# qope/SIPP

Hardware: AMD Instinct MI355X
Metric: SIPP proof-gen wall-clock + pairings-aggregated/sec, n=128 (the 3 STARK sub-proofs, hardened G1/G2 AIRs; outer plonky2 proof not included) (higher is better)
Workload: dtype u64; 1 GPU; n=128 SIPP instance per GPU: G1ExpStark 127 IO (N=2^16, W+P+Q=1176), G2ExpStark 127 IO (N=2^16, 2314), Fq12ExpStark 14 IO (N=2^13, 7970); IO records on host -> 3 flat proofs on host, the 3 sub-proofs on 3 concurrent HIP streams; parallelism=1 independent SIPP instance(s), one per GPU, no collective

## Files before the change

### sipp_amd/csrc/trace.hip

```cpp
#include <algorithm>

#include "air_prog.hpp"
#include "air_tables.h"
#include "ctx.hpp"
#include "fq.hpp"

namespace {

using fq::Fq;
using fq::Fq2;

template <int EXT>
struct Fld;
template <>
struct Fld<1> {
    using T = Fq;
    static __device__ __forceinline__ T add(const T& a, const T& b) { return fq::add(a, b); }
    static __device__ __forceinline__ T sub(const T& a, const T& b) { return fq::sub(a, b); }
    static __device__ __forceinline__ T mul(const T& a, const T& b) { return fq::mul(a, b); }
    static __device__ __forceinline__ T sqr(const T& a) { return fq::sqr(a); }
    static __device__ __forceinline__ T inv(const T& a) { return fq::inv(a); }
    static __device__ __forceinline__ bool is_zero(const T& a) { return fq::is_zero(a); }
    static __device__ __forceinline__ T load(const uint32_t* w) {
        Fq r;
#pragma unroll
        for (int i = 0; i < 8; i++) r.l[i] = w[i];
        return fq::to_mont(r);
    }
};
template <>
struct Fld<2> {
    using T = Fq2;
    static __device__ __forceinline__ T add(const T& a, const T& b) { return fq::add(a, b); }
    static __device__ __forceinline__ T sub(const T& a, const T& b) { return fq::sub(a, b); }
    static __device__ __forceinline__ T mul(const T& a, const T& b) { return fq::mul(a, b); }
    static __device__ __forceinline__ T sqr(const T& a) { return fq::sqr(a); }
    static __device__ __forceinline__ T inv(const T& a) { return fq::inv(a); }
    static __device__ __forceinline__ bool is_zero(const T& a) { return fq::is_zero(a); }
    static __device__ __forceinline__ T load(const uint32_t* w) {
        return Fq2{Fld<1>::load(w), Fld<1>::load(w + 8)};
    }
};

__device__ __forceinline__ Fq one_of(Fq*) { return fq::one_m(); }
__device__ __forceinline__ Fq2 one_of(Fq2*) { return Fq2{fq::one_m(), fq::zero()}; }

template <int EXT>
__device__ __forceinline__ bool point_on_curve(const uint32_t* w) {
    using F = Fld<EXT>;
    const auto x = F::load(w), y = F::load(w + 8 * EXT);
    const auto d = F::sub(F::sqr(y), F::mul(F::sqr(x), x));
    const Fq three = fq::small_m(3);
    if constexpr (EXT == 1) {
        return fq::is_zero(fq::sub(d, three));
    } else {
        const Fq nine = fq::small_m(9);
        const Fq re = fq::sub(fq::mul(nine, d.c0), d.c1), im = fq::add(d.c0, fq::mul(nine, d.c1));
        return fq::is_zero(fq::sub(re, three)) && fq::is_zero(im);
    }
}


template <int EXT>
struct Jac {
    typename Fld<EXT>::T x, y, z;
};

template <int EXT>
__device__ __forceinline__ Jac<EXT> jac_dbl(const Jac<EXT>& p) {
    using F = Fld<EXT>;
    auto A = F::sqr(p.x), B = F::sqr(p.y), C = F::sqr(B);
    auto t = F::add(p.x, B);
    auto D = F::sub(F::sub(F::sqr(t), A), C);
    D = F::add(D, D);
    auto E = F::add(F::add(A, A), A);
    auto Fv = F::sqr(E);
    Jac<EXT> r;
    r.x = F::sub(Fv, F::add(D, D));
    auto C8 = F::add(C, C);
    C8 = F::add(C8, C8);
    C8 = F::add(C8, C8);
    r.y = F::sub(F::mul(E, F::sub(D, r.x)), C8);
    auto yz = F::mul(p.y, p.z);
    r.z = F::add(yz, yz);
    return r;
}

template <int EXT>
__device__ __forceinline__ Jac<EXT> jac_add(const Jac<EXT>& p, const Jac<EXT>& q) {
    using F = Fld<EXT>;
    auto z1z1 = F::sqr(p.z), z2z2 = F::sqr(q.z);
    auto u1 = F::mul(p.x, z2z2), u2 = F::mul(q.x, z1z1);
    auto s1 = F::mul(F::mul(p.y, q.z), z2z2), s2 = F::mul(F::mul(q.y, p.z), z1z1);
    auto h = F::sub(u2, u1);
    auto rr = F::sub(s2, s1);
    if (F::is_zero(h)) {
        if (F::is_zero(rr)) return jac_dbl<EXT>(p);
        Jac<EXT> inf;
        inf.x = one_of((typename F::T*)nullptr);
        inf.y = inf.x;
        inf.z = F::sub(inf.x, inf.x);
        return inf;
    }
    auto i = F::add(h, h);
    i = F::sqr(i);
    auto j = F::mul(h, i);
    rr = F::add(rr, rr);
    auto v = F::mul(u1, i);
    Jac<EXT> r;
    r.x = F::sub(F::sub(F::sqr(rr), j), F::add(v, v));
    auto s1j = F::mul(s1, j);
    r.y = F::sub(F::mul(rr, F::sub(v, r.x)), F::add(s1j, s1j));
    auto zz = F::add(p.z, q.z);
    r.z = F::mul(F::sub(F::sub(F::sqr(zz), z1z1), z2z2), h);
    return r;
}


template <int EXT>
struct RowPts {
    Jac<EXT> R, P;
};

template <int EXT>
__device__ __forceinline__ bool jac_is_inf(const Jac<EXT>& p) { return Fld<EXT>::is_zero(p.z); }

template <int EXT>
__device__ __forceinline__ Jac<EXT> jac_add_id(const Jac<EXT>& p, const Jac<EXT>& q) {
    if (jac_is_inf<EXT>(p)) return q;
    if (jac_is_inf<EXT>(q)) return p;
    return jac_add<EXT>(p, q);
}

__device__ __forceinline__ void lds_put(Fq* dst, const Fq& v) {
    uint4* d = reinterpret_cast<uint4*>(dst);
    d[0] = make_uint4(v.l[0], v.l[1], v.l[2], v.l[3]);
    d[1] = make_uint4(v.l[4], v.l[5], v.l[6], v.l[7]);
}
__device__ __forceinline__ Fq lds_get(const Fq* src) {
    const uint4* d = reinterpret_cast<const uint4*>(src);
    const uint4 a = d[0], b = d[1];
    Fq v;
    v.l[0] = a.x; v.l[1] = a.y; v.l[2] = a.z; v.l[3] = a.w;
    v.l[4] = b.x; v.l[5] = b.y; v.l[6] = b.z; v.l[7] = b.w;
    return v;
}

template <int NT>
__device__ __forceinline__ void par_level(Fq* s_op, Fq* s_pr, int sub, const Fq (&a)[NT], const Fq (&b)[NT], Fq (&p)[NT]) {
#pragma unroll
    for (int t = 0; t < NT; t++) {
        lds_put(s_op + 2 * t, a[t]);
        lds_put(s_op + 2 * t + 1, b[t]);
    }
    __syncthreads();
    const int task = sub < NT ? sub : NT - 1;
    const Fq x = lds_get(s_op + 2 * task), y = lds_get(s_op + 2 * task + 1);
    lds_put(s_pr + sub, fq::mul(x, y));
    __syncthreads();
#pragma unroll
    for (int t = 0; t < NT; t++) p[t] = lds_get(s_pr + t);
}

__device__ __forceinline__ Jac<1> jac_dbl_par(const Jac<1>& P, Fq* s_op, Fq* s_pr, int sub) {
    Fq p1[3], p2[3], p3[1];
    {
        const Fq a[3] = {P.x, P.y, P.y}, b[3] = {P.x, P.y, P.z};
        par_level<3>(s_op, s_pr, sub, a, b, p1);
    }
    const Fq A = p1[0], B = p1[1];
    const Fq U = fq::add(P.x, B), E = fq::add(fq::add(A, A), A);
    {
        const Fq a[3] = {B, U, E};
        par_level<3>(s_op, s_pr, sub, a, a, p2);
    }
    const Fq C = p2[0];
    Fq D = fq::sub(fq::sub(p2[1], A), C);
    D = fq::add(D, D);
    Jac<1> r;
    r.x = fq::sub(p2[2], fq::add(D, D));
    {
        const Fq a[1] = {E}, b[1] = {fq::sub(D, r.x)};
        par_level<1>(s_op, s_pr, sub, a, b, p3);
    }
    Fq C8 = fq::add(C, C);
    C8 = fq::add(C8, C8);
    C8 = fq::add(C8, C8);
    r.y = fq::sub(p3[0], C8);
    r.z = fq::add(p1[2], p1[2]);
    return r;
}

__device__ __forceinline__ Jac<2> jac_dbl_par(const Jac<2>& P, Fq* s_op, Fq* s_pr, int sub) {
    Fq p1[7], p2[6], p3[3];
    {
        const Fq a[7] = {fq::add(P.x.c0, P.x.c1), P.x.c0, fq::add(P.y.c0, P.y.c1), P.y.c0, P.y.c0, P.y.c1,
                         fq::add(P.y.c0, P.y.c1)};
        const Fq b[7] = {fq::sub(P.x.c0, P.x.c1), P.x.c1, fq::sub(P.y.c0, P.y.c1), P.y.c1, P.z.c0, P.z.c1,
                         fq::add(P.z.c0, P.z.c1)};
        par_level<7>(s_op, s_pr, sub, a, b, p1);
    }
    const Fq2 A{p1[0], fq::add(p1[1], p1[1])}, B{p1[2], fq::add(p1[3], p1[3])};
    const Fq2 YZ{fq::sub(p1[4], p1[5]), fq::sub(fq::sub(p1[6], p1[4]), p1[5])};
    const Fq2 U = fq::add(P.x, B), E = fq::add(fq::add(A, A), A);
    {
        const Fq a[6] = {fq::add(B.c0, B.c1), B.c0, fq::add(U.c0, U.c1), U.c0, fq::add(E.c0, E.c1), E.c0};
        const Fq b[6] = {fq::sub(B.c0, B.c1), B.c1, fq::sub(U.c0, U.c1), U.c1, fq::sub(E.c0, E.c1), E.c1};
        par_level<6>(s_op, s_pr, sub, a, b, p2);
    }
    const Fq2 C{p2[0], fq::add(p2[1], p2[1])}, S{p2[2], fq::add(p2[3], p2[3])}, Fv{p2[4], fq::add(p2[5], p2[5])};
    Fq2 D = fq::sub(fq::sub(S, A), C);
    D = fq::add(D, D);
    Jac<2> r;
    r.x = fq::sub(Fv, fq::add(D, D));
    const Fq2 Wd = fq::sub(D, r.x);
    {
        const Fq a[3] = {E.c0, E.c1, fq::add(E.c0, E.c1)}, b[3] = {Wd.c0, Wd.c1, fq::add(Wd.c0, Wd.c1)};
        par_level<3>(s_op, s_pr, sub, a, b, p3);
    }
    const Fq2 EW{fq::sub(p3[0], p3[1]), fq::sub(fq::sub(p3[2], p3[0]), p3[1])};
    Fq2 C8 = fq::add(C, C);
    C8 = fq::add(C8, C8);
    C8 = fq::add(C8, C8);
    r.y = fq::sub(EW, C8);
    r.z = fq::add(YZ, YZ);
    return r;
}

template <int EXT, int G>
__global__ void __launch_bounds__(64) curve_dbl_par_kernel(const uint32_t* __restrict__ ios, uint32_t num_io, uint32_t ppi,
                                                          RowPts<EXT>* __restrict__ rows) {
    using F = Fld<EXT>;
    using T = typename F::T;
    constexpr int GPB = 64 / G;
    __shared__ Fq s_op[GPB][14], s_pr[GPB][G];
    const int grp = threadIdx.x / G, sub = threadIdx.x % G;
    uint32_t io = blockIdx.x * GPB + grp;
    const bool live = io < num_io && sub == 0;
    if (io >= num_io) io = num_io - 1;
    const uint32_t* rec = ios + (size_t)io * ppi;
    const int w = 8 * EXT;
    RowPts<EXT>* out = rows + (size_t)io * 512;
    Jac<EXT> P{F::load(rec), F::load(rec + w), one_of((T*)nullptr)};
    for (int b = 0; b < 256; b++) {
        if (live) out[2 * b].P = P;
        if (b != 255) P = jac_dbl_par(P, s_op[grp], s_pr[grp], sub);
    }
}

template <int EXT>
__global__ void __launch_bounds__(256) curve_scan_kernel(const uint32_t* __restrict__ ios, uint32_t num_io, uint32_t ppi,
                                                        RowPts<EXT>* __restrict__ rows) {
    using F = Fld<EXT>;
    using T = typename F::T;
    __shared__ Jac<EXT> pts[256];
    const uint32_t io = blockIdx.x, k = threadIdx.x;
    const uint32_t* rec = ios + (size_t)io * ppi;
    const int w = 8 * EXT;
    RowPts<EXT>* out = rows + (size_t)io * 512;
    const Jac<EXT> Pk = out[2 * k].P;
    const uint32_t* ex = rec + 4 * w;
    const int bit = (ex[k >> 5] >> (k & 31)) & 1;
    Jac<EXT> inf;
    inf.x = one_of((T*)nullptr);
    inf.y = one_of((T*)nullptr);
    inf.z = F::sub(inf.x, inf.x);
    Jac<EXT> v = bit ? Pk : inf;
    for (int off = 1; off < 256; off <<= 1) {
        pts[k] = v;
        __syncthreads();
        Jac<EXT> o = inf;
        if ((int)k >= off) o = pts[k - off];
        __syncthreads();
        if ((int)k >= off) v = jac_add_id<EXT>(o, v);
    }
    const Jac<EXT> offs{F::load(rec + 2 * w), F::load(rec + 3 * w), one_of((T*)nullptr)};
    const Jac<EXT> A = jac_add_id<EXT>(offs, v);
    pts[k] = A;
    __syncthreads();
    const Jac<EXT> Rk = k ? pts[k - 1] : offs;
    out[2 * k].R = Rk;
    out[2 * k + 1].R = A;
    out[2 * k + 1].P = Pk;
}

__device__ __forceinline__ void store_limbs16(uint64_t* tr, size_t n, int col, size_t row, const Fq& std_form) {
#pragma unroll
    for (int i = 0; i < 8; i++) {
        tr[(size_t)(col + 2 * i) * n + row] = std_form.l[i] & 0xffffu;
        tr[(size_t)(col + 2 * i + 1) * n + row] = std_form.l[i] >> 16;
    }
}
__device__ __forceinline__ void store_checked(uint64_t* tr, size_t n, int col, size_t row, const Fq& std_form, int cpl) {
    if (cpl == 1) {
        store_limbs16(tr, n, col, row, std_form);
    } else {
#pragma unroll
        for (int i = 0; i < 8; i++) {
            uint32_t v = std_form.l[i];
            tr[(size_t)(col + 4 * i) * n + row] = v & 0xffu;
            tr[(size_t)(col + 4 * i + 1) * n + row] = (v >> 8) & 0xffu;
            tr[(size_t)(col + 4 * i + 2) * n + row] = (v >> 16) & 0xffu;
            tr[(size_t)(col + 4 * i + 3) * n + row] = v >> 24;
        }
    }
}
template <int EXT>
__device__ __forceinline__ void store_f_u16(uint64_t* tr, size_t n, int col, size_t row, const typename Fld<EXT>::T& v);
template <>
__device__ __forceinline__ void store_f_u16<1>(uint64_t* tr, size_t n, int col, size_t row, const Fq& v) {
    store_limbs16(tr, n, col, row, fq::from_mont(v));
}
template <>
__device__ __forceinline__ void store_f_u16<2>(uint64_t* tr, size_t n, int col, size_t row, const Fq2& v) {
    store_limbs16(tr, n, col, row, fq::from_mont(v.c0));
    store_limbs16(tr, n, col + 16, row, fq::from_mont(v.c1));
}
template <int EXT>
__device__ __forceinline__ void store_f_chk(uint64_t* tr, size_t n, int col, size_t row, const typename Fld<EXT>::T& v,
                                            int cpl);
template <>
__device__ __forceinline__ void store_f_chk<1>(uint64_t* tr, size_t n, int col, size_t row, const Fq& v, int cpl) {
    store_checked(tr, n, col, row, fq::from_mont(v), cpl);
}
template <>
__device__ __forceinline__ void store_f_chk<2>(uint64_t* tr, size_t n, int col, size_t row, const Fq2& v, int cpl) {
    store_checked(tr, n, col, row, fq::from_mont(v.c0), cpl);
    store_checked(tr, n, col + 16 * cpl, row, fq::from_mont(v.c1), cpl);
}
// ... 597 lines not shown
        int32_t va[16], vb[16];
        w += ivec_dev<16>(w, tr, n, row, per, g, va, bad);
        bool live = false;
#pragma unroll
        for (int i = 0; i < 16; i++) live |= va[i] != 0;
        if (!live) continue;
        (void)ivec_dev<16>(w, tr, n, row, per, g, vb, bad);
#pragma unroll
        for (int i = 0; i < 16; i++) {
            const int64_t a64 = coef * va[i];
            const int32_t ai = (int32_t)a64;
            bad |= a64 != (int64_t)ai;
#pragma unroll
            for (int j = 0; j < 16; j++) e[i + j] += (int64_t)ai * vb[j];
        }
    }
#pragma unroll
    for (int i = 0; i < 31; i++) {
        long long v = e[i];
#pragma unroll
        for (int d = 32; d >= 1; d >>= 1) v += __shfl_xor(v, d, 64);
        e[i] = v;
    }
    if (lane == 0) {
#pragma unroll
        for (int i = 0; i < 31; i++) g.esum[row * 32 + (size_t)i] = e[i];
    }
    if (bad) atomicExch(err, SIPP_E_WITNESS);
}

__global__ void hist_kernel(const uint64_t* __restrict__ cols, size_t n, uint32_t ncols, uint32_t tbits,
                            uint32_t* __restrict__ hist) {
    size_t total = n * ncols;
    for (size_t i = (size_t)blockIdx.x * blockDim.x + threadIdx.x; i < total; i += (size_t)gridDim.x * blockDim.x) {
        size_t c = i / n;
        uint64_t v = cols[i];
        atomicAdd(&hist[(c << tbits) + (v & (((uint64_t)1 << tbits) - 1))], 1u);
    }
}

constexpr uint32_t HIST16_BINS = 16384, HIST16_PARTS = 65536 / HIST16_BINS, HIST16_SHIFT = 14;
__global__ void __launch_bounds__(1024) hist_u16_kernel(const uint64_t* __restrict__ cols, size_t n, uint32_t* __restrict__ hist) {
    extern __shared__ uint32_t hs[];
    for (uint32_t i = threadIdx.x; i < HIST16_BINS; i += 1024) hs[i] = 0;
    __syncthreads();
    const size_t c = blockIdx.z;
    const uint32_t part = blockIdx.y;
    const uint64_t* col = cols + c * n;
    const size_t chunk = (n + gridDim.x - 1) / gridDim.x, lo = blockIdx.x * chunk, hi = min(n, lo + chunk);
    for (size_t i0 = lo; i0 < hi; i0 += 1024) {
        const size_t i = i0 + threadIdx.x;
        const bool live = i < hi;
        const uint32_t v = live ? (uint32_t)col[i] & 0xffffu : 0xffffffffu;
        const uint32_t v0 = __builtin_amdgcn_readfirstlane(v);
        if (__all(v == v0)) {
            if (v0 != 0xffffffffu && (v0 >> HIST16_SHIFT) == part && (threadIdx.x & 63) == 0) atomicAdd(&hs[v0 & (HIST16_BINS - 1)], 64u);
        } else if (live && (v >> HIST16_SHIFT) == part) {
            atomicAdd(&hs[v & (HIST16_BINS - 1)], 1u);
        }
    }
    __syncthreads();
    uint32_t* out = hist + (c << 16) + ((size_t)part << HIST16_SHIFT);
    for (uint32_t i = threadIdx.x; i < HIST16_BINS; i += 1024) {
        const uint32_t x = hs[i];
        if (x) {
            if (gridDim.x == 1) out[i] = x;
            else atomicAdd(&out[i], x);
        }
    }
}

__global__ void __launch_bounds__(256) hist_u8_kernel(const uint64_t* __restrict__ cols, size_t n, uint32_t* __restrict__ hist) {
    __shared__ uint32_t h[256];
    h[threadIdx.x] = 0;
    __syncthreads();
    const size_t c = blockIdx.y;
    const uint64_t* col = cols + c * n;
    const size_t chunk = (n + gridDim.x - 1) / gridDim.x, lo = blockIdx.x * chunk, hi = min(n, lo + chunk);
    for (size_t i = lo + threadIdx.x; i < hi; i += 256) atomicAdd(&h[col[i] & 0xff], 1u);
    __syncthreads();
    if (h[threadIdx.x]) atomicAdd(&hist[(c << 8) + threadIdx.x], h[threadIdx.x]);
}

__global__ void __launch_bounds__(256) lookup_scan_kernel(const uint32_t* __restrict__ hist, uint32_t tbits,
                                                         uint32_t* __restrict__ start, uint32_t* __restrict__ dist,
                                                         uint32_t* __restrict__ zlist, uint32_t* __restrict__ nzero) {
    __shared__ uint32_t s_cnt[256], s_dst[256], s_zer[256];
    const uint32_t T = 1u << tbits, per = T / 256;
    const size_t c = blockIdx.x;
    const uint32_t* h = hist + (c << tbits);
    uint32_t* st = start + (c << tbits);
    uint32_t* ds = dist + (c << tbits);
    uint32_t* zl = zlist + (c << tbits);
    const uint32_t v0 = threadIdx.x * per;
    uint32_t cnt = 0, dst = 0, zer = 0;
    if (per % 4 == 0) {
        const uint4* h4 = reinterpret_cast<const uint4*>(h + v0);
#pragma unroll 8
        for (uint32_t k = 0; k < per / 4; k++) {
            const uint4 x = h4[k];
            cnt += x.x + x.y + x.z + x.w;
            const uint32_t nz = (x.x != 0) + (x.y != 0) + (x.z != 0) + (x.w != 0);
            dst += nz;
            zer += 4 - nz;
        }
    } else {
        for (uint32_t v = v0; v < v0 + per; v++) {
            uint32_t x = h[v];
            cnt += x;
            dst += x != 0;
            zer += x == 0;
        }
    }
    s_cnt[threadIdx.x] = cnt;
    s_dst[threadIdx.x] = dst;
    s_zer[threadIdx.x] = zer;
    __syncthreads();
    if (threadIdx.x == 0) {
        uint32_t a = 0, b = 0, z = 0;
        for (int i = 0; i < 256; i++) {
            uint32_t ta = s_cnt[i], tb = s_dst[i], tz = s_zer[i];
            s_cnt[i] = a;
            s_dst[i] = b;
            s_zer[i] = z;
            a += ta;
            b += tb;
            z += tz;
        }
        nzero[c] = z;
    }
    __syncthreads();
    cnt = s_cnt[threadIdx.x];
    dst = s_dst[threadIdx.x];
    zer = s_zer[threadIdx.x];
    if (per % 4 == 0) {
        const uint4* h4 = reinterpret_cast<const uint4*>(h + v0);
        uint4* st4 = reinterpret_cast<uint4*>(st + v0);
        uint4* ds4 = reinterpret_cast<uint4*>(ds + v0);
#pragma unroll 4
        for (uint32_t k = 0; k < per / 4; k++) {
            const uint4 x = h4[k];
            const uint32_t v = v0 + 4 * k;
            uint4 so, dd;
            so.x = cnt; cnt += x.x; dst += x.x != 0; dd.x = dst; if (x.x == 0) zl[zer++] = v;
            so.y = cnt; cnt += x.y; dst += x.y != 0; dd.y = dst; if (x.y == 0) zl[zer++] = v + 1;
            so.z = cnt; cnt += x.z; dst += x.z != 0; dd.z = dst; if (x.z == 0) zl[zer++] = v + 2;
            so.w = cnt; cnt += x.w; dst += x.w != 0; dd.w = dst; if (x.w == 0) zl[zer++] = v + 3;
            st4[k] = so;
            ds4[k] = dd;
        }
    } else {
        for (uint32_t v = v0; v < v0 + per; v++) {
            uint32_t x = h[v];
            st[v] = cnt;
            cnt += x;
            dst += x != 0;
            ds[v] = dst;
            if (x == 0) zl[zer++] = v;
        }
    }
}

__global__ void __launch_bounds__(256) lookup_expand_kernel(const uint32_t* __restrict__ hist, const uint32_t* __restrict__ start,
                                                           const uint32_t* __restrict__ dist, const uint32_t* __restrict__ zlist,
                                                           const uint32_t* __restrict__ nzero, size_t n, uint32_t tbits,
                                                           uint64_t* __restrict__ pin, uint64_t* __restrict__ ptab) {
    const uint32_t T = 1u << tbits;
    const size_t c = blockIdx.y;
    const uint32_t v = blockIdx.x * blockDim.x + threadIdx.x;
    const bool live = v < T;
    const size_t tb = (c << tbits);
    const uint32_t cnt = live ? hist[tb + v] : 0, s = live ? start[tb + v] : 0, d = live ? dist[tb + v] : 0;
    const uint32_t nz = nzero[c];
    const uint32_t* zl = zlist + tb;
    uint64_t* pi = pin + c * n;
    uint64_t* pt = ptab + c * n;
    const uint32_t LIGHT = 8;
    if (cnt && cnt <= LIGHT) {
        pi[s] = v;
        pt[s] = v;
        for (uint32_t j = 1; j < cnt; j++) {
            const uint32_t i = s + j, k = i - d;
            pi[i] = v;
            pt[i] = k < nz ? zl[k] : T - 1;
        }
    }
    uint64_t heavy = __ballot(cnt > LIGHT);
    const uint32_t lane = threadIdx.x & 63;
    while (heavy) {
        const int src = __ffsll((unsigned long long)heavy) - 1;
        heavy &= heavy - 1;
        const uint32_t hv = __shfl(v, src), hs = __shfl(s, src), hc = __shfl(cnt, src), hd = __shfl(d, src);
        uint32_t j = lane;
        for (; j + 7 * 64 < hc; j += 8 * 64) {
            uint32_t f[8];
#pragma unroll
            for (int q = 0; q < 8; q++) {
                const uint32_t k = hs + j + 64 * q - hd;
                f[q] = k < nz ? zl[k] : T - 1;
            }
#pragma unroll
            for (int q = 0; q < 8; q++) {
                const uint32_t i = hs + j + 64 * q;
                pi[i] = hv;
                pt[i] = (j + 64 * q) == 0 ? hv : f[q];
            }
        }
        for (; j < hc; j += 64) {
            const uint32_t i = hs + j, k = i - hd;
            pi[i] = hv;
            pt[i] = j == 0 ? hv : (k < nz ? zl[k] : T - 1);
        }
    }
}

}

const air_spec_t* sipp_air_get(int kind, uint32_t log_n) {
    const bool u16 = log_n >= 16;
    if (kind < 0 || kind > 6) return nullptr;
    const int hard = (kind == 4 || kind == 5) ? 1 : 0, base = hard ? kind - 4 : kind;
    for (size_t i = 0; i < sizeof(AIR_AIRS) / sizeof(AIR_AIRS[0]); i++)
        if (AIR_AIRS[i].kind == base && AIR_AIRS[i].hardened == hard && (AIR_AIRS[i].table_bits == 16) == u16) return &AIR_AIRS[i];
    return nullptr;
}

static int64_t* prog_on_device(sipp_ctx* ctx, const air_spec_t* a) {
    uint64_t* t = sipp_table_get(ctx, TAB_AIR_PROG, (uint64_t)(a->kind + 8 * a->hardened), (uint64_t)a->table_bits);
    if (t) return (int64_t*)t;
    std::vector<uint64_t> v(a->prog_len);
    memcpy(v.data(), a->prog, (size_t)a->prog_len * 8);
    if (sipp_table_put(ctx, TAB_AIR_PROG, (uint64_t)(a->kind + 8 * a->hardened), (uint64_t)a->table_bits, v, &t) != SIPP_OK) return nullptr;
    return (int64_t*)t;
}
const int64_t* sipp_air_prog_device(sipp_ctx* ctx, const air_spec_t* a) { return prog_on_device(ctx, a); }
const int8_t* sipp_air_vflag_device(sipp_ctx* ctx, const air_spec_t* a) {
    if (a->n_vflag == 0) return nullptr;
    uint64_t* t = sipp_table_get(ctx, TAB_VFLAG, (uint64_t)a->kind, 0);
    if (!t) {
        const size_t bytes = (size_t)a->n_vflag << a->log_rows;
        std::vector<uint64_t> v((bytes + 7) / 8, 0);
        int8_t* f = reinterpret_cast<int8_t*>(v.data());
        for (int k = 0; k < a->n_vflag; k++)
            for (int r = 0; r < (1 << a->log_rows); r++) f[((size_t)k << a->log_rows) + (size_t)r] = (int8_t)air_vper_value(a, k, r);
        if (sipp_table_put(ctx, TAB_VFLAG, (uint64_t)a->kind, 0, v, &t) != SIPP_OK) return nullptr;
    }
    return reinterpret_cast<const int8_t*>(t);
}

template <int EXT>
static void curve_dbl(hipStream_t st, const uint32_t* d_ios, uint32_t num_io, uint32_t ppi, void* rows) {
    constexpr uint32_t PER = 16 / EXT;
    hipLaunchKernelGGL((curve_dbl_par_kernel<EXT, 4 * EXT>), dim3((num_io + PER - 1) / PER), dim3(64), 0, st, d_ios, num_io, ppi,
                       reinterpret_cast<RowPts<EXT>*>(rows));
}
template <int EXT>
static void curve_scan(hipStream_t st, const uint32_t* d_ios, uint32_t num_io, uint32_t ppi, void* rows) {
    hipLaunchKernelGGL(curve_scan_kernel<EXT>, dim3(num_io), dim3(256), 0, st, d_ios, num_io, ppi, reinterpret_cast<RowPts<EXT>*>(rows));
}
template <int EXT>
static void curve_outputs(hipStream_t st, void* rows, uint32_t* d_ios, uint32_t num_io, uint32_t ppi, int* d_err) {
    hipLaunchKernelGGL(curve_outputs_kernel<EXT>, dim3((num_io + 63) / 64), dim3(64), 0, st, reinterpret_cast<RowPts<EXT>*>(rows), d_ios,
                       num_io, ppi, d_err);
}

size_t sipp_fold_rows_bytes(int kind, uint32_t num_io) {
    return (size_t)num_io * 512 * (kind == 0 ? sizeof(RowPts<1>) : sizeof(RowPts<2>));
}
int sipp_fold_chain_begin(sipp_ctx* ctx, int kind, const uint32_t* d_ios, uint32_t num_io, uint32_t ppi, void* rows, hipStream_t st) {
    (kind == 0 ? curve_dbl<1> : curve_dbl<2>)(st, d_ios, num_io, ppi, rows);
    SIPP_CHECK_HIP(ctx, hipGetLastError());
    return SIPP_OK;
}
int sipp_fold_chain_finish(sipp_ctx* ctx, int kind, uint32_t* d_ios, uint32_t num_io, uint32_t ppi, void* rows, int* d_err,
                           hipStream_t st) {
    if (kind == 0) {
        curve_scan<1>(st, d_ios, num_io, ppi, rows);
        curve_outputs<1>(st, rows, d_ios, num_io, ppi, d_err);
    } else {
        curve_scan<2>(st, d_ios, num_io, ppi, rows);
        curve_outputs<2>(st, rows, d_ios, num_io, ppi, d_err);
    }
    SIPP_CHECK_HIP(ctx, hipGetLastError());
    return SIPP_OK;
}

static void gate_after_chain(sipp_ctx* ctx) {
    if (ctx->gate_wait) {
        ctx->gate_wait->wait();
        ctx->gate_wait = nullptr;
    }
}

static const int32_t* hard_layout(const air_spec_t* a) {
    if (!a->hardened || a->kind > 1) return nullptr;
    return a->kind == 0 ? (a->cells_per_limb == 1 ? AIR_HARD_LAYOUT_G1H_U16 : AIR_HARD_LAYOUT_G1H_U8)
                        : (a->cells_per_limb == 1 ? AIR_HARD_LAYOUT_G2H_U16 : AIR_HARD_LAYOUT_G2H_U8);
}

static int fq12_chain(sipp_ctx* ctx, const air_spec_t* a, const uint32_t* d_ios, uint32_t num_io, uint64_t* d_trace, size_t n) {
    Fq12Cols c{1, 1 + 192, a->checked_base, a->cells_per_limb};
    ProfScope ps(ctx, "trace_fq12_chain");
    hipLaunchKernelGGL(fq12_chain_kernel, dim3(num_io), dim3(384), 0, ctx->stream, d_ios, num_io, d_trace, n, c);
    SIPP_CHECK_HIP(ctx, hipGetLastError());
    return SIPP_OK;
}

template <int EXT>
static int curve_trace(sipp_ctx* ctx, const air_spec_t* a, const uint32_t* d_ios, uint32_t num_io, size_t n, int hard_inf_col,
                       uint64_t* d_trace, int* d_err) {
    const int ncl = 16 * EXT, cpl = a->cells_per_limb;
    CurveCols c{1, 1 + ncl, 1 + 2 * ncl, 1 + 3 * ncl, a->checked_base, a->checked_base + ncl * cpl, a->checked_base + 2 * ncl * cpl, cpl};
    RowPts<EXT>* rows = arena_alloc_t<RowPts<EXT>>(ctx, n);
    if (!rows) return SIPP_E_NOMEM;
    {
        ProfScope ps(ctx, "trace_curve_chain");
        curve_dbl<EXT>(ctx->stream, d_ios, num_io, (uint32_t)a->pi_per_io, rows);
        curve_scan<EXT>(ctx->stream, d_ios, num_io, (uint32_t)a->pi_per_io, rows);
    }
    SIPP_CHECK_HIP(ctx, hipGetLastError());
    gate_after_chain(ctx);
    ProfScope ps(ctx, "trace_curve_rows");
    hipLaunchKernelGGL(curve_rows_kernel<EXT>, dim3((unsigned)(n / ROWS_BLOCK)), dim3(ROWS_BLOCK), 0, ctx->stream, rows, d_trace, n, c,
                       a->hardened, hard_inf_col, d_err);
    SIPP_CHECK_HIP(ctx, hipGetLastError());
    return SIPP_OK;
}

int sipp_outputs_fill(sipp_ctx* ctx, const air_spec_t* a, uint32_t* d_ios, uint32_t num_io, uint32_t log_n, int* d_err) {
    const size_t n = (size_t)1 << log_n;
    const uint32_t ppi = (uint32_t)a->pi_per_io;
    if (a->kind == 3) return sipp_mapg2_outputs(ctx, d_ios, num_io, d_err);
    if (a->kind == 6) return sipp_pairing_outputs(ctx, d_ios, num_io, d_err);
    ArenaScope scope(ctx);
    if (a->kind == 2) {
        uint64_t* d_trace = arena_alloc_t<uint64_t>(ctx, (size_t)(a->n_main + 2 * a->n_checked) << log_n);
// ... 160 lines not shown
```

Baseline: 2512 pairings/s.

## Use lazy-reduced 29-bit limb chain for curve doubling and tile the lookup scan

Replaces the cooperative Jacobian doubling with a 9x29-bit unsaturated-limb representation where adds and subs skip modular reduction. Each doubling becomes three fused multiply levels, with the lanes writing canonical outputs directly to the row buffer. The G2 group widens from 8 to 16 lanes. Separately, the lookup scan kernel replaces its serial thread-0 prefix pass with tiled wave-shuffle scans and prefetch. The intent is to shorten the serial doubling chain and remove a serial scan bottleneck, at the cost of relying on hand-tuned limb-bound slack for correctness.

```diff
diff --git a/sipp_amd/csrc/fq_chain.hpp b/sipp_amd/csrc/fq_chain.hpp
--- /dev/null
+++ b/sipp_amd/csrc/fq_chain.hpp
@@ -0,0 +1,253 @@
+#pragma once
+#include <stdint.h>
+
+#if defined(__HIPCC__)
+#include <hip/hip_runtime.h>
+#define FQC_HD __host__ __device__ __forceinline__
+#else
+#define FQC_HD inline
+#endif
+
+namespace fqc {
+
+constexpr uint32_t P29[9] = {0x187cfd47u, 0x010460b6u, 0x1c72a34fu, 0x02d522d0u, 0x1585d978u,
+                             0x02db40c0u, 0x00a6e141u, 0x0e5c2634u, 0x0030644eu};
+constexpr uint32_t NINV29 = 0x04866389u;
+constexpr uint32_t M29 = (1u << 29) - 1;
+constexpr uint32_t ONE29[9] = {0x157ccc21u, 0x141c2758u, 0x185230d3u, 0x014c0419u, 0x0aa36fb9u,
+                               0x1d4240ceu, 0x11d54c07u, 0x052ac7a8u, 0x000dc836u};
+constexpr uint32_t P32[8] = {0xd87cfd47u, 0x3c208c16u, 0x6871ca8du, 0x97816a91u, 0x8181585du, 0xb85045b6u, 0xe131a029u, 0x30644e72u};
+
+struct L9 {
+    uint32_t l[9];
+};
+
+struct Off {
+    uint32_t l[9];
+};
+constexpr Off make_off(uint32_t c, uint32_t w) {
+    Off o{};
+    uint64_t carry = 0;
+    for (int i = 0; i < 9; i++) {
+        const uint64_t t = (uint64_t)P29[i] * c + carry;
+        o.l[i] = i < 8 ? (uint32_t)(t & M29) : (uint32_t)t;
+        carry = t >> 29;
+    }
+    o.l[0] += w << 29;
+    for (int i = 1; i < 8; i++) o.l[i] += (w << 29) - w;
+    o.l[8] -= w;
+    return o;
+}
+FQC_HD L9 add(const L9& a, const L9& b) {
+    L9 r;
+#if defined(__HIP_DEVICE_COMPILE__)
+#pragma unroll
+#endif
+    for (int i = 0; i < 9; i++) r.l[i] = a.l[i] + b.l[i];
+    return r;
+}
+FQC_HD L9 dbl(const L9& a) { return add(a, a); }
+template <uint32_t C, uint32_t W>
+FQC_HD L9 sub(const L9& a, const L9& b) {
+    constexpr Off k = make_off(C, W);
+    L9 r;
+#if defined(__HIP_DEVICE_COMPILE__)
+#pragma unroll
+#endif
+    for (int i = 0; i < 9; i++) r.l[i] = (a.l[i] + k.l[i]) - b.l[i];
+    return r;
+}
+FQC_HD L9 norm1(const L9& a) {
+    L9 r;
+    r.l[0] = a.l[0] & M29;
+#if defined(__HIP_DEVICE_COMPILE__)
+#pragma unroll
+#endif
+    for (int i = 1; i < 8; i++) r.l[i] = (a.l[i] & M29) + (a.l[i - 1] >> 29);
+    r.l[8] = a.l[8] + (a.l[7] >> 29);
+    return r;
+}
+
+FQC_HD L9 mul(const L9& x, const L9& y) {
+    uint32_t m[9];
+    L9 r;
+    uint64_t acc = 0;
+#if defined(__HIP_DEVICE_COMPILE__)
+#pragma unroll
+#endif
+    for (int k = 0; k < 17; k++) {
+#if defined(__HIP_DEVICE_COMPILE__)
+#pragma unroll
+#endif
+        for (int i = 0; i < 9; i++) {
+            const int j = k - i;
+            if (j >= 0 && j < 9) acc += (uint64_t)x.l[i] * y.l[j];
+        }
+#if defined(__HIP_DEVICE_COMPILE__)
+#pragma unroll
+#endif
+        for (int i = 0; i < 9; i++) {
+            const int j = k - i;
+            if (i < k && j >= 0 && j < 9) acc += (uint64_t)m[i] * P29[j];
+        }
+        if (k < 9) {
+            m[k] = ((uint32_t)acc * NINV29) & M29;
+            acc += (uint64_t)m[k] * P29[0];
+        } else {
+            r.l[k - 9] = (uint32_t)acc & M29;
+        }
+        acc >>= 29;
+    }
+    r.l[8] = (uint32_t)acc;
+    return r;
+}
+
+FQC_HD L9 cut(const uint32_t (&a)[8]) {
+    L9 o;
+#if defined(__HIP_DEVICE_COMPILE__)
+#pragma unroll
+#endif
+    for (int k = 0; k < 9; k++) {
+        const int w = (29 * k) >> 5, sh = (29 * k) & 31;
+        uint32_t v = a[w] >> sh;
+        if (sh > 3 && w < 7) v |= a[w + 1] << (32 - sh);
+        o.l[k] = v & M29;
+    }
+    return o;
+}
+FQC_HD void canon_words(uint32_t (&o)[8], const L9& r) {
+    uint32_t j32[8], d[8];
+#if defined(__HIP_DEVICE_COMPILE__)
+#pragma unroll
+#endif
+    for (int j = 0; j < 8; j++) {
+        const int k = (32 * j) / 29, sh = 32 * j - 29 * k;
+        uint32_t v = r.l[k] >> sh;
+        v |= r.l[k + 1] << (29 - sh);
+        if (58 - sh < 32 && k + 2 < 9) v |= r.l[k + 2] << (58 - sh);
+        j32[j] = v;
+    }
+    uint32_t bw = 0;
+#if defined(__HIP_DEVICE_COMPILE__)
+#pragma unroll
+#endif
+    for (int i = 0; i < 8; i++) {
+#if defined(__HIP_DEVICE_COMPILE__)
+        d[i] = __builtin_subc(j32[i], P32[i], bw, &bw);
+#else
+        const uint64_t t = (uint64_t)j32[i] - P32[i] - bw;
+        d[i] = (uint32_t)t;
+        bw = (uint32_t)(t >> 32) & 1u;
+#endif
+    }
+#if defined(__HIP_DEVICE_COMPILE__)
+#pragma unroll
+#endif
+    for (int i = 0; i < 8; i++) o[i] = bw ? j32[i] : d[i];
+}
+constexpr uint32_t NEG8_29[9] = {0x1d9096cdu, 0x022be75eu, 0x12c66350u, 0x1e1f47a4u, 0x0b760e9fu,
+                                 0x1e7fbbcfu, 0x134a4383u, 0x01be3557u, 0x0022eb3au};
+FQC_HD L9 neg8() {
+    L9 r;
+#if defined(__HIP_DEVICE_COMPILE__)
+#pragma unroll
+#endif
+    for (int i = 0; i < 9; i++) r.l[i] = NEG8_29[i];
+    return r;
+}
+FQC_HD L9 one() {
+    L9 r;
+#if defined(__HIP_DEVICE_COMPILE__)
+#pragma unroll
+#endif
+    for (int i = 0; i < 9; i++) r.l[i] = ONE29[i];
+    return r;
+}
+
+template <class T, class Lv>
+FQC_HD void dbl_g2(T (&X)[2], T (&Y)[2], T (&Z)[2], const T& one_v, const T& neg8_v, Lv& lv) {
+    lv.chk("X0", X[0], 1, 120); lv.chk("X1", X[1], 1, 120); lv.chk("Z0", Z[0], 1, 120); lv.chk("Z1", Z[1], 1, 120);
+    lv.chk("Y0", Y[0], 2, 600); lv.chk("Y1", Y[1], 2, 600);
+    T p1[8], p2[8], p3[8];
+    {
+        const T v[13] = {add(X[0], X[1]), sub<2, 1>(X[0], X[1]), dbl(X[0]), X[1], add(Y[0], Y[1]), sub<7, 2>(Y[0], Y[1]),
+                         dbl(Y[0]), Y[1], dbl(Y[1]), Z[0], Z[1], Y[0], one_v};
+        lv.template level<13, 8>(1, v, 0x7777777b86866420ull, 0xcccccccc9aa97531ull, p1, 8, 2, 16);
+    }
+    const T A0 = p1[0], A1 = p1[1], B0 = p1[2], B1 = p1[3];
+    lv.chk("A0", A0, 1, 110); lv.chk("A1", A1, 1, 110); lv.chk("B0", B0, 1, 200); lv.chk("B1", B1, 1, 150);
+    lv.chk("T4", p1[4], 1, 110); lv.chk("T5", p1[5], 1, 110); lv.chk("T6", p1[6], 1, 110); lv.chk("T7", p1[7], 1, 110);
+    const T Zl0 = sub<2, 1>(p1[4], p1[5]), Zl1 = add(p1[6], p1[7]);
+    lv.chk("Zl0", Zl0, 3, 310); lv.chk("Zl1", Zl1, 2, 220);
+    const T U0 = add(X[0], B0), U1 = add(X[1], B1);
+    const T E0 = add(dbl(A0), A0), E1 = add(dbl(A1), A1);
+    lv.chk("U0", U0, 2, 320); lv.chk("U1", U1, 2, 270); lv.chk("E0", E0, 3, 330); lv.chk("E1", E1, 3, 330);
+    {
+        const T v[15] = {add(B0, B1), sub<2, 1>(B0, B1), dbl(B0), B1, add(U0, U1), sub<3, 2>(U0, U1), dbl(U0), U1,
+                         add(E0, E1), sub<4, 3>(E0, E1), dbl(E0), E1, Zl0, Zl1, one_v};
+        lv.template level<15, 8>(2, v, 0xdddddddddca86420ull, 0xeeeeeeeeeeb97531ull, p2, 6, 2, 32);
+    }
+    const T C0 = p2[0], C1 = p2[1], S0 = p2[2], S1 = p2[3], F0 = p2[4], F1 = p2[5];
+    lv.chk("C0", C0, 1, 120); lv.chk("C1", C1, 1, 120); lv.chk("S0", S0, 1, 130); lv.chk("S1", S1, 1, 130);
+    lv.chk("F0", F0, 1, 140); lv.chk("F1", F1, 1, 140);
+    const T G0 = add(A0, C0), G1 = add(A1, C1);
+    lv.chk("G0", G0, 2, 230); lv.chk("G1", G1, 2, 230);
+    const T Dh0 = sub<3, 2>(S0, G0), Dh1 = sub<3, 2>(S1, G1);
+    lv.chk("Dh0", Dh0, 4, 430); lv.chk("Dh1", Dh1, 4, 430);
+    const T D20 = dbl(norm1(Dh0)), D21 = dbl(norm1(Dh1));
+    const T D40 = dbl(D20), D41 = dbl(D21);
+    lv.chk("D40", D40, 5, 1720); lv.chk("D41", D41, 5, 1720);
+    const T Xl0 = sub<18, 5>(F0, D40), Xl1 = sub<18, 5>(F1, D41);
+    lv.chk("Xl0", Xl0, 7, 1940); lv.chk("Xl1", Xl1, 7, 1940);
+    const T Wd0 = add(norm1(sub<2, 1>(D20, F0)), D40), Wd1 = add(norm1(sub<2, 1>(D21, F1)), D41);
+    lv.chk("Wd0", Wd0, 6, 2780); lv.chk("Wd1", Wd1, 6, 2780);
+    {
+        const T v[10] = {E0, E1, Wd0, Wd1, Xl0, Xl1, C0, C1, one_v, neg8_v};
+        lv.template level<10, 8>(3, v, 0x7777777776541010ull, 0x9999999999882332ull, p3, 4, 2, 0);
+    }
+    lv.chk("r0", p3[0], 1, 160); lv.chk("r1", p3[1], 1, 160); lv.chk("r2", p3[2], 1, 160); lv.chk("r3", p3[3], 1, 160);
+    lv.chk("n0", p3[6], 1, 110); lv.chk("n1", p3[7], 1, 110);
+    X[0] = p3[4]; X[1] = p3[5]; Z[0] = p2[6]; Z[1] = p2[7];
+    Y[0] = norm1(add(sub<2, 1>(p3[0], p3[1]), p3[6]));
+    Y[1] = norm1(add(add(p3[2], p3[3]), p3[7]));
+    lv.chk("X0'", X[0], 1, 120); lv.chk("X1'", X[1], 1, 120); lv.chk("Z0'", Z[0], 1, 120); lv.chk("Z1'", Z[1], 1, 120);
+    lv.chk("Y0'", Y[0], 2, 600); lv.chk("Y1'", Y[1], 2, 600);
+}
+
+template <class T, class Lv>
+FQC_HD void dbl_g1(T& X, T& Y, T& Z, const T& one_v, const T& neg8_v, Lv& lv) {
+    lv.chk("X", X, 1, 120); lv.chk("Z", Z, 1, 120); lv.chk("Y", Y, 2, 600);
+    T p1[3], p2[4], p3[3];
+    {
+        const T v[5] = {X, Y, dbl(Y), Z, one_v};
+        lv.template level<5, 3>(1, v, 0x1210ull, 0x4310ull, p1, 3, 1, 8);
+    }
+    const T A = p1[0], B = p1[1], Zl = p1[2];
+    lv.chk("A", A, 1, 110); lv.chk("B", B, 1, 130); lv.chk("Zl", Zl, 1, 110);
+    const T U = add(X, B), E = add(dbl(A), A);
+    lv.chk("U", U, 2, 250); lv.chk("E", E, 3, 330);
+    {
+        const T v[5] = {B, U, E, Zl, one_v};
+        lv.template level<5, 4>(2, v, 0x3210ull, 0x4210ull, p2, 3, 1, 16);
+    }
+    const T C = p2[0], S = p2[1], F = p2[2];
+    lv.chk("C", C, 1, 110); lv.chk("S", S, 1, 110); lv.chk("F", F, 1, 110);
+    const T G = add(A, C);
+    const T Dh = sub<3, 2>(S, G);
+    lv.chk("Dh", Dh, 4, 410);
+    const T D2 = dbl(norm1(Dh)), D4 = dbl(D2);
+    const T Xl = sub<17, 5>(F, D4);
+    const T Wd = add(norm1(sub<2, 1>(D2, F)), D4);
+    lv.chk("Xl", Xl, 7, 1810); lv.chk("Wd", Wd, 6, 2650);
+    {
+        const T v[6] = {E, Wd, Xl, C, one_v, neg8_v};
+        lv.template level<6, 3>(3, v, 0x3320ull, 0x5541ull, p3, 1, 1, 0);
+    }
+    lv.chk("r", p3[0], 1, 160); lv.chk("n", p3[2], 1, 110);
+    X = p3[1];
+    Z = p2[3];
+    Y = norm1(add(p3[0], p3[2]));
+    lv.chk("X'", X, 1, 120); lv.chk("Z'", Z, 1, 120); lv.chk("Y'", Y, 2, 600);
+}
+
+}
diff --git a/sipp_amd/csrc/trace.hip b/sipp_amd/csrc/trace.hip
--- a/sipp_amd/csrc/trace.hip
+++ b/sipp_amd/csrc/trace.hip
@@ -4,6 +4,7 @@
 #include "air_tables.h"
 #include "ctx.hpp"
 #include "fq.hpp"
+#include "fq_chain.hpp"
 
 namespace {
 
@@ -132,119 +133,103 @@
     return jac_add<EXT>(p, q);
 }
 
-__device__ __forceinline__ void lds_put(Fq* dst, const Fq& v) {
+__device__ __forceinline__ void lds_put9(uint32_t* dst, const fqc::L9& v) {
     uint4* d = reinterpret_cast<uint4*>(dst);
     d[0] = make_uint4(v.l[0], v.l[1], v.l[2], v.l[3]);
     d[1] = make_uint4(v.l[4], v.l[5], v.l[6], v.l[7]);
-}
-__device__ __forceinline__ Fq lds_get(const Fq* src) {
+    dst[8] = v.l[8];
+}
+__device__ __forceinline__ fqc::L9 lds_get9(const uint32_t* src) {
     const uint4* d = reinterpret_cast<const uint4*>(src);
     const uint4 a = d[0], b = d[1];
-    Fq v;
+    fqc::L9 v;
     v.l[0] = a.x; v.l[1] = a.y; v.l[2] = a.z; v.l[3] = a.w;
     v.l[4] = b.x; v.l[5] = b.y; v.l[6] = b.z; v.l[7] = b.w;
+    v.l[8] = src[8];
     return v;
 }
 
-template <int NT>
-__device__ __forceinline__ void par_level(Fq* s_op, Fq* s_pr, int sub, const Fq (&a)[NT], const Fq (&b)[NT], Fq (&p)[NT]) {
-#pragma unroll
-    for (int t = 0; t < NT; t++) {
-        lds_put(s_op + 2 * t, a[t]);
-        lds_put(s_op + 2 * t + 1, b[t]);
-    }
-    __syncthreads();
-    const int task = sub < NT ? sub : NT - 1;
-    const Fq x = lds_get(s_op + 2 * task), y = lds_get(s_op + 2 * task + 1);
-    lds_put(s_pr + sub, fq::mul(x, y));
-    __syncthreads();
-#pragma unroll
-    for (int t = 0; t < NT; t++) p[t] = lds_get(s_pr + t);
-}
-
-__device__ __forceinline__ Jac<1> jac_dbl_par(const Jac<1>& P, Fq* s_op, Fq* s_pr, int sub) {
-    Fq p1[3], p2[3], p3[1];
-    {
-        const Fq a[3] = {P.x, P.y, P.y}, b[3] = {P.x, P.y, P.z};
-        par_level<3>(s_op, s_pr, sub, a, b, p1);
-    }
-    const Fq A = p1[0], B = p1[1];
-    const Fq U = fq::add(P.x, B), E = fq::add(fq::add(A, A), A);
-    {
-        const Fq a[3] = {B, U, E};
-        par_level<3>(s_op, s_pr, sub, a, a, p2);
-    }
-    const Fq C = p2[0];
-    Fq D = fq::sub(fq::sub(p2[1], A), C);
-    D = fq::add(D, D);
-    Jac<1> r;
-    r.x = fq::sub(p2[2], fq::add(D, D));
-    {
-        const Fq a[1] = {E}, b[1] = {fq::sub(D, r.x)};
-        par_level<1>(s_op, s_pr, sub, a, b, p3);
-    }
-    Fq C8 = fq::add(C, C);
-    C8 = fq::add(C8, C8);
-    C8 = fq::add(C8, C8);
-    r.y = fq::sub(p3[0], C8);
-    r.z = fq::add(p1[2], p1[2]);
-    return r;
-}
-
-__device__ __forceinline__ Jac<2> jac_dbl_par(const Jac<2>& P, Fq* s_op, Fq* s_pr, int sub) {
-    Fq p1[7], p2[6], p3[3];
-    {
-        const Fq a[7] = {fq::add(P.x.c0, P.x.c1), P.x.c0, fq::add(P.y.c0, P.y.c1), P.y.c0, P.y.c0, P.y.c1,
-                         fq::add(P.y.c0, P.y.c1)};
-        const Fq b[7] = {fq::sub(P.x.c0, P.x.c1), P.x.c1, fq::sub(P.y.c0, P.y.c1), P.y.c1, P.z.c0, P.z.c1,
-                         fq::add(P.z.c0, P.z.c1)};
-        par_level<7>(s_op, s_pr, sub, a, b, p1);
-    }
-    const Fq2 A{p1[0], fq::add(p1[1], p1[1])}, B{p1[2], fq::add(p1[3], p1[3])};
-    const Fq2 YZ{fq::sub(p1[4], p1[5]), fq::sub(fq::sub(p1[6], p1[4]), p1[5])};
-    const Fq2 U = fq::add(P.x, B), E = fq::add(fq::add(A, A), A);
-    {
-        const Fq a[6] = {fq::add(B.c0, B.c1), B.c0, fq::add(U.c0, U.c1), U.c0, fq::add(E.c0, E.c1), E.c0};
-        const Fq b[6] = {fq::sub(B.c0, B.c1), B.c1, fq::sub(U.c0, U.c1), U.c1, fq::sub(E.c0, E.c1), E.c1};
-        par_level<6>(s_op, s_pr, sub, a, b, p2);
-    }
-    const Fq2 C{p2[0], fq::add(p2[1], p2[1])}, S{p2[2], fq::add(p2[3], p2[3])}, Fv{p2[4], fq::add(p2[5], p2[5])};
-    Fq2 D = fq::sub(fq::sub(S, A), C);
-    D = fq::add(D, D);
-    Jac<2> r;
-    r.x = fq::sub(Fv, fq::add(D, D));
-    const Fq2 Wd = fq::sub(D, r.x);
-    {
-        const Fq a[3] = {E.c0, E.c1, fq::add(E.c0, E.c1)}, b[3] = {Wd.c0, Wd.c1, fq::add(Wd.c0, Wd.c1)};
-        par_level<3>(s_op, s_pr, sub, a, b, p3);
-    }
-    const Fq2 EW{fq::sub(p3[0], p3[1]), fq::sub(fq::sub(p3[2], p3[0]), p3[1])};
-    Fq2 C8 = fq::add(C, C);
-    C8 = fq::add(C8, C8);
-    C8 = fq::add(C8, C8);
-    r.y = fq::sub(EW, C8);
-    r.z = fq::add(YZ, YZ);
-    return r;
-}
+constexpr int CHAIN_SLOTS = 16, CHAIN_SLOT_WORDS = 12;
+struct ChainLevels {
+    uint32_t* s_val;
+    uint32_t* s_pr;
+    int sub;
+    uint32_t* cur;
+    uint32_t* next;
+    __device__ __forceinline__ void chk(const char*, const fqc::L9&, uint32_t, uint32_t) const {}
+    template <int NV, int NP>
+    __device__ __forceinline__ void level(int id, const fqc::L9 (&v)[NV], uint64_t ia, uint64_t ib, fqc::L9 (&p)[NP], int st_lane,
+                                          int st_cnt, int st_off) const {
+        static_assert(NV <= CHAIN_SLOTS, "operand slots");
+#pragma unroll
+        for (int t = 0; t < NV; t++) lds_put9(s_val + CHAIN_SLOT_WORDS * t, v[t]);
+        __syncthreads();
+        const uint32_t sa = (uint32_t)(ia >> (4 * sub)) & 15u, sb = (uint32_t)(ib >> (4 * sub)) & 15u;
+        const fqc::L9 a = fqc::norm1(lds_get9(s_val + CHAIN_SLOT_WORDS * sa)), b = fqc::norm1(lds_get9(s_val + CHAIN_SLOT_WORDS * sb));
+        const fqc::L9 r = fqc::mul(a, b);
+        lds_put9(s_pr + CHAIN_SLOT_WORDS * sub, r);
+        uint32_t* pt = id == 1 ? cur : next;
+        if (pt && sub >= st_lane && sub < st_lane + st_cnt) {
+            uint32_t w[8];
+            fqc::canon_words(w, r);
+            uint32_t* d = pt + st_off + 8 * (sub - st_lane);
+#pragma unroll
+            for (int i = 0; i < 8; i++) d[i] = w[i];
+        }
+        __syncthreads();
+#pragma unroll
+        for (int t = 0; t < NP; t++) p[t] = lds_get9(s_pr + CHAIN_SLOT_WORDS * t);
+    }
+};
 
 template <int EXT, int G>
 __global__ void __launch_bounds__(64) curve_dbl_par_kernel(const uint32_t* __restrict__ ios, uint32_t num_io, uint32_t ppi,
                                                           RowPts<EXT>* __restrict__ rows) {
     using F = Fld<EXT>;
     using T = typename F::T;
+    using fqc::L9;
     constexpr int GPB = 64 / G;
-    __shared__ Fq s_op[GPB][14], s_pr[GPB][G];
+    static_assert(sizeof(Jac<EXT>) == 3 * 8 * EXT * sizeof(uint32_t), "the levels store a point's coordinates by word offset");
+    __shared__ __attribute__((aligned(16))) uint32_t s_val[GPB][CHAIN_SLOTS * CHAIN_SLOT_WORDS], s_pr[GPB][G * CHAIN_SLOT_WORDS];
     const int grp = threadIdx.x / G, sub = threadIdx.x % G;
     uint32_t io = blockIdx.x * GPB + grp;
-    const bool live = io < num_io && sub == 0;
+    const bool live = io < num_io;
     if (io >= num_io) io = num_io - 1;
     const uint32_t* rec = ios + (size_t)io * ppi;
     const int w = 8 * EXT;
     RowPts<EXT>* out = rows + (size_t)io * 512;
-    Jac<EXT> P{F::load(rec), F::load(rec + w), one_of((T*)nullptr)};
-    for (int b = 0; b < 256; b++) {
-        if (live) out[2 * b].P = P;
-        if (b != 255) P = jac_dbl_par(P, s_op[grp], s_pr[grp], sub);
+    const T x0 = F::load(rec), y0 = F::load(rec + w);
+    if (live && sub == 0) {
+        out[0].P.x = x0;
+        out[0].P.z = one_of((T*)nullptr);
+    }
+    const L9 one = fqc::one(), n8 = fqc::neg8();
+    ChainLevels lv{s_val[grp], s_pr[grp], sub, nullptr, nullptr};
+    if constexpr (EXT == 1) {
+        L9 X = fqc::cut(x0.l), Y = fqc::cut(y0.l), Z = one;
+        for (int b = 0; b < 255; b++) {
+            lv.cur = live ? reinterpret_cast<uint32_t*>(&out[2 * b].P) : nullptr;
+            lv.next = live ? reinterpret_cast<uint32_t*>(&out[2 * b + 2].P) : nullptr;
+            fqc::dbl_g1(X, Y, Z, one, n8, lv);
+        }
+        lv.cur = live ? reinterpret_cast<uint32_t*>(&out[510].P) : nullptr;
+        const L9 v[2] = {Y, one};
+        L9 unused[1];
+        lv.template level<2, 1>(1, v, 0x0000ull, 0x1111ull, unused, 0, 1, 8);
+    } else {
+        L9 X[2] = {fqc::cut(x0.c0.l), fqc::cut(x0.c1.l)}, Y[2] = {fqc::cut(y0.c0.l), fqc::cut(y0.c1.l)};
+        L9 Z[2] = {one, one};
+#pragma unroll
+        for (int i = 0; i < 9; i++) Z[1].l[i] = 0;
+        for (int b = 0; b < 255; b++) {
+            lv.cur = live ? reinterpret_cast<uint32_t*>(&out[2 * b].P) : nullptr;
+            lv.next = live ? reinterpret_cast<uint32_t*>(&out[2 * b + 2].P) : nullptr;
+            fqc::dbl_g2(X, Y, Z, one, n8, lv);
+        }
+        lv.cur = live ? reinterpret_cast<uint32_t*>(&out[510].P) : nullptr;
+        const L9 v[3] = {Y[0], Y[1], one};
+        L9 unused[1];
+        lv.template level<3, 1>(1, v, 0x1111111111111110ull, 0x2222222222222222ull, unused, 0, 2, 16);
     }
 }
 
@@ -1008,83 +993,91 @@
     if (h[threadIdx.x]) atomicAdd(&hist[(c << 8) + threadIdx.x], h[threadIdx.x]);
 }
 
+template <int VEC>
+__device__ __forceinline__ void lookup_scan_tiles(const uint32_t* __restrict__ h, uint32_t T, uint32_t* __restrict__ st,
+                                                  uint32_t* __restrict__ ds, uint32_t* __restrict__ zl, uint32_t (&s_tot)[2][2][4],
+                                                  uint32_t& run_dst) {
+    const uint32_t lane = threadIdx.x & 63, wv = threadIdx.x >> 6, tiles = T / (256 * VEC);
+    uint32_t run_cnt = 0;
+    uint32_t x[VEC], nx[VEC];
+    auto load = [&](uint32_t (&o)[VEC], uint32_t tile) {
+        if constexpr (VEC == 4) {
+            const uint4 q = reinterpret_cast<const uint4*>(h)[tile * 256 + threadIdx.x];
+            o[0] = q.x; o[1] = q.y; o[2] = q.z; o[3] = q.w;
+        } else {
+            o[0] = h[tile * 256 + threadIdx.x];
+        }
+    };
+    load(x, 0);
+    for (uint32_t tile = 0; tile < tiles; tile++) {
+        if (tile + 1 < tiles) load(nx, tile + 1);
+        uint32_t c4 = 0, n4 = 0;
+#pragma unroll
+        for (int k = 0; k < VEC; k++) {
+            c4 += x[k];
+            n4 += x[k] != 0;
+        }
+        uint32_t ic = c4, in = n4;
+#pragma unroll
+        for (int d = 1; d < 64; d <<= 1) {
+            const uint32_t tc = __shfl_up(ic, d, 64), tn = __shfl_up(in, d, 64);
+            if ((int)lane >= d) {
+                ic += tc;
+                in += tn;
+            }
+        }
+        if (lane == 63) {
+            s_tot[tile & 1][0][wv] = ic;
+            s_tot[tile & 1][1][wv] = in;
+        }
+        __syncthreads();
+        uint32_t cnt = run_cnt + ic - c4, dst = run_dst + in - n4;
+#pragma unroll
+        for (uint32_t q = 0; q < 4; q++) {
+            const uint32_t a = s_tot[tile & 1][0][q], b = s_tot[tile & 1][1][q];
+            if (q < wv) {
+                cnt += a;
+                dst += b;
+            }
+            run_cnt += a;
+            run_dst += b;
+        }
+        const uint32_t v = (tile * 256 + threadIdx.x) * VEC;
+        uint32_t zer = v - dst;
+        uint32_t so[VEC], dd[VEC];
+#pragma unroll
+        for (int k = 0; k < VEC; k++) {
+            so[k] = cnt;
+            cnt += x[k];
+            dst += x[k] != 0;
+            dd[k] = dst;
+            if (x[k] == 0) zl[zer++] = v + k;
+        }
+        if constexpr (VEC == 4) {
+            reinterpret_cast<uint4*>(st)[tile * 256 + threadIdx.x] = make_uint4(so[0], so[1], so[2], so[3]);
+            reinterpret_cast<uint4*>(ds)[tile * 256 + threadIdx.x] = make_uint4(dd[0], dd[1], dd[2], dd[3]);
+        } else {
+            st[v] = so[0];
+            ds[v] = dd[0];
+        }
+#pragma unroll
+        for (int k = 0; k < VEC; k++) x[k] = nx[k];
+    }
+}
 __global__ void __launch_bounds__(256) lookup_scan_kernel(const uint32_t* __restrict__ hist, uint32_t tbits,
                                                          uint32_t* __restrict__ start, uint32_t* __restrict__ dist,
                                                          uint32_t* __restrict__ zlist, uint32_t* __restrict__ nzero) {
-    __shared__ uint32_t s_cnt[256], s_dst[256], s_zer[256];
-    const uint32_t T = 1u << tbits, per = T / 256;
+    __shared__ uint32_t s_tot[2][2][4];
+    const uint32_t T = 1u << tbits;
     const size_t c = blockIdx.x;
     const uint32_t* h = hist + (c << tbits);
     uint32_t* st = start + (c << tbits);
     uint32_t* ds = dist + (c << tbits);
     uint32_t* zl = zlist + (c << tbits);
-    const uint32_t v0 = threadIdx.x * per;
-    uint32_t cnt = 0, dst = 0, zer = 0;
-    if (per % 4 == 0) {
-        const uint4* h4 = reinterpret_cast<const uint4*>(h + v0);
-#pragma unroll 8
-        for (uint32_t k = 0; k < per / 4; k++) {
-            const uint4 x = h4[k];
-            cnt += x.x + x.y + x.z + x.w;
-            const uint32_t nz = (x.x != 0) + (x.y != 0) + (x.z != 0) + (x.w != 0);
-            dst += nz;
-            zer += 4 - nz;
-        }
-    } else {
-        for (uint32_t v = v0; v < v0 + per; v++) {
-            uint32_t x = h[v];
-            cnt += x;
-            dst += x != 0;
-            zer += x == 0;
-        }
-    }
-    s_cnt[threadIdx.x] = cnt;
-    s_dst[threadIdx.x] = dst;
-    s_zer[threadIdx.x] = zer;
-    __syncthreads();
-    if (threadIdx.x == 0) {
-        uint32_t a = 0, b = 0, z = 0;
-        for (int i = 0; i < 256; i++) {
-            uint32_t ta = s_cnt[i], tb = s_dst[i], tz = s_zer[i];
-            s_cnt[i] = a;
-            s_dst[i] = b;
-            s_zer[i] = z;
-            a += ta;
-            b += tb;
-            z += tz;
-        }
-        nzero[c] = z;
-    }
-    __syncthreads();
-    cnt = s_cnt[threadIdx.x];
-    dst = s_dst[threadIdx.x];
-    zer = s_zer[threadIdx.x];
-    if (per % 4 == 0) {
-        const uint4* h4 = reinterpret_cast<const uint4*>(h + v0);
-        uint4* st4 = reinterpret_cast<uint4*>(st + v0);
-        uint4* ds4 = reinterpret_cast<uint4*>(ds + v0);
-#pragma unroll 4
-        for (uint32_t k = 0; k < per / 4; k++) {
-            const uint4 x = h4[k];
-            const uint32_t v = v0 + 4 * k;
-            uint4 so, dd;
-            so.x = cnt; cnt += x.x; dst += x.x != 0; dd.x = dst; if (x.x == 0) zl[zer++] = v;
-            so.y = cnt; cnt += x.y; dst += x.y != 0; dd.y = dst; if (x.y == 0) zl[zer++] = v + 1;
-            so.z = cnt; cnt += x.z; dst += x.z != 0; dd.z = dst; if (x.z == 0) zl[zer++] = v + 2;
-            so.w = cnt; cnt += x.w; dst += x.w != 0; dd.w = dst; if (x.w == 0) zl[zer++] = v + 3;
-            st4[k] = so;
-            ds4[k] = dd;
-        }
-    } else {
-        for (uint32_t v = v0; v < v0 + per; v++) {
-            uint32_t x = h[v];
-            st[v] = cnt;
-            cnt += x;
-            dst += x != 0;
-            ds[v] = dst;
-            if (x == 0) zl[zer++] = v;
-        }
-    }
+    uint32_t distinct = 0;
+    if (T % 1024 == 0) lookup_scan_tiles<4>(h, T, st, ds, zl, s_tot, distinct);
+    else lookup_scan_tiles<1>(h, T, st, ds, zl, s_tot, distinct);
+    if (threadIdx.x == 0) nzero[c] = T - distinct;
 }
 
 __global__ void __launch_bounds__(256) lookup_expand_kernel(const uint32_t* __restrict__ hist, const uint32_t* __restrict__ start,
@@ -1176,8 +1169,8 @@
 
 template <int EXT>
 static void curve_dbl(hipStream_t st, const uint32_t* d_ios, uint32_t num_io, uint32_t ppi, void* rows) {
-    constexpr uint32_t PER = 16 / EXT;
-    hipLaunchKernelGGL((curve_dbl_par_kernel<EXT, 4 * EXT>), dim3((num_io + PER - 1) / PER), dim3(64), 0, st, d_ios, num_io, ppi,
+    constexpr uint32_t G = EXT == 1 ? 4 : 16, PER = 64 / G;
+    hipLaunchKernelGGL((curve_dbl_par_kernel<EXT, G>), dim3((num_io + PER - 1) / PER), dim3(64), 0, st, d_ios, num_io, ppi,
                        reinterpret_cast<RowPts<EXT>*>(rows));
 }
 template <int EXT>
```

New measurement: 2531 pairings/s, median of 6. About the same (+0.8%).
